# tum-vision/pnec

Hardware: AMD Instinct MI355X
Metric: PNEC pose solves/sec (512 corr, 10 GN iters) (higher is better)
Workload: dtype f64; 1 GPU; configs[1]: batch of 100k simulated frame pairs x 512 anisotropic-covariance correspondences per GPU; pairs_total=100000, launcher=single process, residual=PNEC target frame, setup_launches_before_warmup=15, pairs_per_gpu=100000, correspondences=512

## Files before the change

### pnec_amd/csrc/pnec_capi.hip

```cpp
#include <hip/hip_runtime.h>

#include <algorithm>
#include <cmath>
#include <cstdio>
#include <cstdlib>
#include <cstring>
#include <new>
#include <string>
#include <vector>

#include "pnec_batch_kernels.hpp"
#include "pnec_device.hpp"
#include "pnec_detect.hpp"
#include "pnec_front_shared.hpp"
#include "pnec_internal.hpp"
#include "pnec_keyframe.hpp"
#include "pnec_patch_cov.hpp"
#include "pnec_patch_store.hpp"
#include "pnec_patch_track.hpp"
#include "pnec_pose_cov.hpp"
#include "pnec_residuals.hpp"
#include "pnec_eight_point.hpp"
#include "pnec_undistort.hpp"
#include "pnec_trajectory.hpp"
// ... 526 lines not shown
    const std::string msg = g_last_error;
    pnec_hip_problem_destroy(p);
    g_last_error = msg;
    return rc;
  }
  *out = p;
  return 0;
}

int pnec_hip_problem_create(int device, int mode, int64_t n_pairs, const int64_t *offsets,
                            pnec_hip_problem **out) {
  return problem_create_impl(device, mode, 0, 0, n_pairs, offsets, out);
}

int pnec_hip_problem_create_capacity(int device, int mode, int64_t max_pairs, int64_t max_corr,
                                     pnec_hip_problem **out) {
  if (!out) return fail(PNEC_HIP_ERR_INVALID_ARGUMENT, "out is NULL");
  *out = nullptr;
  if (mode < PNEC_HIP_MODE_NEC || mode > PNEC_HIP_MODE_SYM) return fail(PNEC_HIP_ERR_INVALID_ARGUMENT, "unknown mode");
  if (max_pairs < 1 || max_corr < 0 || max_corr > (int64_t)1 << 40)
    return fail(PNEC_HIP_ERR_INVALID_ARGUMENT, "need max_pairs >= 1, max_corr >= 0");
  const int64_t cap_doubles = (int64_t)num_components(mode) * ((max_corr + 63 * max_pairs + kWave - 1) & ~(int64_t)(kWave - 1));
  const int64_t zero = 0;
  return problem_create_impl(device, mode, max_pairs, cap_doubles, 0, &zero, out);
}

int pnec_hip_problem_reshape(pnec_hip_problem *p, int64_t n_pairs, const int64_t *offsets, void *stream_) {
  return problem_reshape_impl(p, n_pairs, offsets, (hipStream_t)stream_, true);
}

int pnec_hip_problem_destroy(pnec_hip_problem *p) {
  if (!p) return 0;
  DeviceGuard guard(p->device);
  const bool drained = hipDeviceSynchronize() == hipSuccess;
  auto release = [&](void *ptr) { (void)(drained ? dev_free_drained(ptr) : dev_free(ptr)); };
  for (pnec_hip_problem *v : p->chunk_views) pnec_hip_problem_destroy(v);
  for (pnec_hip_problem *v : p->chunk_sel_views) pnec_hip_problem_destroy(v);
  if (p->sel_view) pnec_hip_problem_destroy(p->sel_view);
  if (p->nec_view) pnec_hip_problem_destroy(p->nec_view);
  release(p->d_mask);
  if (p->owns_data) {
    release(p->d_data);
    if (p->d_meta) {
      release(p->d_meta);
    } else {
      release(p->d_block_offset);
      release(p->d_offsets);
      release(p->d_count);
    }
  }
  release(p->d_stage);
  release(p->d_stage_i);
  release(p->d_ratio);
  release(p->d_front);
  release(p->d_front_i);
  release(p->d_hint_its);
  release(p->d_order);
  for (hipStream_t st : p->side_streams) {
    if (drained) pool_stream_put(st, p->device); else (void)hipStreamDestroy(st);
  }
  for (hipEvent_t ev : p->side_done) {
    if (drained) pool_event_put(ev, p->device); else (void)hipEventDestroy(ev);
  }
  for (hipStream_t st : p->chunk_streams) {
    if (drained) pool_stream_put(st, p->device); else (void)hipStreamDestroy(st);
  }
  for (hipEvent_t ev : p->chunk_done) {
    if (drained) pool_event_put(ev, p->device); else (void)hipEventDestroy(ev);
  }
  if (p->fork_event) {
    if (drained) pool_event_put(p->fork_event, p->device); else (void)hipEventDestroy(p->fork_event);
  }
  if (p->meta_uploaded) {
    if (drained) pool_event_put(p->meta_uploaded, p->device); else (void)hipEventDestroy(p->meta_uploaded);
  }
  if (p->bound_uploaded) {
    if (drained) pool_event_put(p->bound_uploaded, p->device); else (void)hipEventDestroy(p->bound_uploaded);
  }
  release(p->d_bound);
  release(p->d_bucket_pairs);
  release(p->d_fill);
  delete p;
  return 0;
}

int pnec_hip_problem_fill(pnec_hip_problem *p, int64_t first_pair, int64_t n_pairs,
                          const double *bvs1, const double *bvs2, const double *covs,
                          const double *covs_host, int space, void *stream_) {
  if (!p) return fail(PNEC_HIP_ERR_INVALID_ARGUMENT, "problem is NULL");
  if (first_pair < 0 || n_pairs < 0 || first_pair + n_pairs > p->n_pairs)
    return fail(PNEC_HIP_ERR_INVALID_ARGUMENT, "pair range out of bounds");
  if (n_pairs == 0) return 0;
  if (int rc = materialize(p)) return rc;
  const int64_t m = p->offsets[(size_t)(first_pair + n_pairs)] - p->offsets[(size_t)first_pair];
  if (m > 0 && (!bvs1 || !bvs2)) return fail(PNEC_HIP_ERR_INVALID_ARGUMENT, "bvs1/bvs2 is NULL");
  if (m > 0 && p->nc >= 12 && !covs)
    return fail(PNEC_HIP_ERR_INVALID_ARGUMENT, "covs is NULL for a PNEC-mode problem");
  if (m > 0 && p->nc >= 18 && !covs_host)
    return fail(PNEC_HIP_ERR_INVALID_ARGUMENT, "covs_host is NULL for a SYM-mode problem");
  DeviceGuard guard(p->device);
  hipStream_t stream = (hipStream_t)stream_;

  const double *d_b1 = bvs1, *d_b2 = bvs2, *d_c = covs, *d_ch = covs_host;
  double *tmp = nullptr;
  bool persistent_stage = false;
  if (space == PNEC_HIP_MEM_HOST && m > 0) {
// ... 297 lines not shown
  PNEC_HIP_TRY(launch_trajectory_metrics(a, stream));
  return io.finish();
}

int64_t pnec_hip_problem_payload_doubles(const pnec_hip_problem *p) { return p ? p->data_doubles : 0; }

int pnec_hip_problem_export_payload(const pnec_hip_problem *p, double *out, int space, void *stream_) {
  if (!p || !out) return fail(PNEC_HIP_ERR_INVALID_ARGUMENT, "NULL argument");
  if (space != PNEC_HIP_MEM_DEVICE && space != PNEC_HIP_MEM_HOST)
    return fail(PNEC_HIP_ERR_INVALID_ARGUMENT, "bad memory space");
  if (p->data_doubles == 0) return 0;
  DeviceGuard guard(p->device);
  hipStream_t stream = (hipStream_t)stream_;
  PNEC_HIP_TRY(hipMemcpyAsync(out, p->d_data, sizeof(double) * p->data_doubles,
                              space == PNEC_HIP_MEM_HOST ? hipMemcpyDeviceToHost : hipMemcpyDeviceToDevice, stream));
  if (space == PNEC_HIP_MEM_HOST) PNEC_HIP_TRY(hipStreamSynchronize(stream));
  return 0;
}

int64_t pnec_hip_problem_num_pairs(const pnec_hip_problem *p) { return p ? p->n_pairs : 0; }
int64_t pnec_hip_problem_num_correspondences(const pnec_hip_problem *p) {
  return p && materialize(p) == 0 ? p->n_corr : 0;
}
int64_t pnec_hip_problem_max_correspondences(const pnec_hip_problem *p) {
  return p && materialize(p) == 0 ? p->n_max : 0;
}
int64_t pnec_hip_problem_payload_bytes(const pnec_hip_problem *p) {
  return p && materialize(p) == 0 ? p->n_corr * p->nc * (int64_t)sizeof(double) : 0;
}
int pnec_hip_problem_offsets(const pnec_hip_problem *p, int64_t *out) {
  if (!p || !out) return fail(PNEC_HIP_ERR_INVALID_ARGUMENT, "NULL argument");
  if (int rc = materialize(p)) return rc;
  std::memcpy(out, p->offsets.data(), sizeof(int64_t) * p->offsets.size());
  return 0;
}
int pnec_hip_problem_mode(const pnec_hip_problem *p) { return p ? p->mode : -1; }
int pnec_hip_problem_device(const pnec_hip_problem *p) { return p ? p->device : -1; }

int pnec_hip_describe_launch(const pnec_hip_problem *p, const pnec_hip_options *opt,
                             int32_t *corr_per_lane, int32_t *waves_per_pair,
                             int32_t *lds_corr_per_lane, int32_t *threads_per_block,
                             int32_t *resident) {
  if (!p) return fail(PNEC_HIP_ERR_INVALID_ARGUMENT, "problem is NULL");
  Geometry g;
  if (int rc = choose_geometry(p, opt, &g)) return rc;
  if (corr_per_lane) *corr_per_lane = g.cpl;
  if (waves_per_pair) *waves_per_pair = g.wpp;
  if (lds_corr_per_lane) *lds_corr_per_lane = g.ldsk;
  if (threads_per_block) *threads_per_block = kWave * g.wpp;
  if (resident) *resident = g.resident ? 1 : 0;
  return 0;
}

int pnec_hip_solve(pnec_hip_problem *p, const double *init_q, const double *init_t, int32_t n_hyp,
                   const double *hyp_t, double reg, const pnec_hip_options *opt_in, double *out_q,
                   double *out_t, double *out_cost, int32_t *out_iterations, int32_t *out_status,
                   int space, void *stream_) {
  if (!p) return fail(PNEC_HIP_ERR_INVALID_ARGUMENT, "problem is NULL");
  if (!init_q) return fail(PNEC_HIP_ERR_INVALID_ARGUMENT, "init_q is NULL");
  if (!hyp_t) n_hyp = 1;
  if (n_hyp < 1) return fail(PNEC_HIP_ERR_INVALID_ARGUMENT, "n_hyp must be >= 1");
  if (!hyp_t && !init_t) return fail(PNEC_HIP_ERR_INVALID_ARGUMENT, "init_t and hyp_t are both NULL");
  if (int rc = check_space("", space)) return rc;
  pnec_hip_options opt;
  if (opt_in)
    opt = *opt_in;
  else
    pnec_hip_default_options(&opt);
  if (opt.max_num_iterations < 0) return fail(PNEC_HIP_ERR_INVALID_ARGUMENT, "max_num_iterations < 0");
  if (opt.flags & ~(PNEC_HIP_OPT_COUNT_PASSES | PNEC_HIP_OPT_JACOBIAN_NUMERIC_CENTRAL))
    return fail(PNEC_HIP_ERR_INVALID_ARGUMENT, "pnec_hip_options.flags: undefined bit set");
  const bool numeric = (opt.flags & PNEC_HIP_OPT_JACOBIAN_NUMERIC_CENTRAL) != 0;
  if (numeric) {
    opt.corr_per_lane = 0;
    opt.waves_per_pair = kStreamWaves;
    opt.lds_corr_per_lane = 0;
  }
  int64_t S;
  if (int rc = pose_slots(p, n_hyp, "solves", &S)) return rc;
  if (S == 0) return 0;
  Geometry g;
  if (int rc = choose_geometry(p, &opt, &g)) return rc;

  hipStream_t stream = (hipStream_t)stream_;
  CallArrays io(p, space, stream);
  SolveArgs a;
  std::memset(&a, 0, sizeof(a));
  a.data = p->d_data;
  a.block_offset = p->d_block_offset;
  a.count = p->d_count;
  a.n_solves = S;
  a.n_hyp = n_hyp;
  a.reg = reg;
  a.opt = opt;
  finish_args(a);
  a.numeric_jacobian = numeric ? 1 : 0;
  if (opt.flags & PNEC_HIP_OPT_COUNT_PASSES) {
    if (int rc = solve_work_buffer(p->device, &a.work)) return rc;
  }

  const int64_t P = p->n_pairs;
  io.in(a.init_q, init_q, 4 * P);
  io.in(a.init_t, init_t, 3 * P);
  io.in(a.hyp_t, hyp_t, 3 * S);
  io.out(a.out_q, out_q, 4 * S, kKeep);
  io.out(a.out_t, out_t, 3 * S, kKeep);
  io.out(a.out_cost, out_cost, S, kKeep);
  io.out(a.out_iterations, out_iterations, S, kKeep);
  io.out(a.out_status, out_status, S, kKeep);
  if (int rc = io.commit()) return rc;

  static const bool use_groups = [] {
    const char *ev = std::getenv("PNEC_SOLVE_GROUPS");
    return !(ev && *ev == '0');
  }();
  auto launch_on = [&](const Geometry &gg, const SolveArgs &aa, hipStream_t st) -> hipError_t {
    if (use_groups && aa.n_hyp > 1 && gg.resident && !aa.trace && !aa.numeric_jacobian &&
        (gg.wpp >= 2 ? group_geometry_ok(p->mode, gg.cpl, gg.wpp, gg.ldsk)
                     : pairhyp_geometry_ok(p->mode, gg.cpl, gg.wpp, gg.ldsk))) {
      switch (p->mode) {
        case PNEC_HIP_MODE_NEC: return launch_solve_group_mode_0(gg.cpl, gg.wpp, gg.ldsk, aa, st);
        case PNEC_HIP_MODE_TARGET: return launch_solve_group_mode_1(gg.cpl, gg.wpp, gg.ldsk, aa, st);
        case PNEC_HIP_MODE_HOST: return launch_solve_group_mode_2(gg.cpl, gg.wpp, gg.ldsk, aa, st);
        default: return launch_solve_group_mode_3(gg.cpl, gg.wpp, gg.ldsk, aa, st);
      }
    }
    switch (p->mode) {
      case PNEC_HIP_MODE_NEC: return launch_solve_mode_0(gg.cpl, gg.wpp, gg.ldsk, gg.resident, aa, st);
      case PNEC_HIP_MODE_TARGET: return launch_solve_mode_1(gg.cpl, gg.wpp, gg.ldsk, gg.resident, aa, st);
      case PNEC_HIP_MODE_HOST: return launch_solve_mode_2(gg.cpl, gg.wpp, gg.ldsk, gg.resident, aa, st);
      default: return launch_solve_mode_3(gg.cpl, gg.wpp, gg.ldsk, gg.resident, aa, st);
    }
  };
  auto launch = [&](const Geometry &gg, const SolveArgs &aa) -> hipError_t { return launch_on(gg, aa, stream); };
  const char *trace_path = std::getenv("PNEC_HIP_TRACE");
  unsigned long long *d_trace = nullptr;
  const bool forced = opt.corr_per_lane > 0 || opt.waves_per_pair > 0;
  if (!forced) {
    if (int rc = ensure_buckets(p)) return rc;
  }
  if (trace_path && *trace_path) {
    PNEC_HIP_TRY(dev_alloc(&d_trace, sizeof(unsigned long long) * 4 * S));
    const hipError_t te = hipMemsetAsync(d_trace, 0, sizeof(unsigned long long) * 4 * S, stream);
    if (te != hipSuccess) {
      (void)dev_free(d_trace);
      return fail_hip(te, "hipMemsetAsync(trace)");
    }
    a.trace = d_trace;
  }
  hipError_t e = hipSuccess;
  if (forced || p->buckets.size() <= 1) {
    e = launch(g, a);
  } else {
    const size_t n_side = p->buckets.size() - 1;
    if (int rc = ensure_side_streams(p, n_side)) {
      if (d_trace) (void)dev_free(d_trace);
      return rc;
    }
    e = hipEventRecord(p->fork_event, stream);
    for (size_t b = 0; b < p->buckets.size() && e == hipSuccess; ++b) {
      const auto &bk = p->buckets[b];
      SolveArgs ab = a;
      ab.pair_index = p->d_bucket_pairs + bk.first;
// ... 1307 lines not shown
```

### pnec_amd/csrc/pnec_internal.hpp

```cpp
#pragma once

#include <hip/hip_runtime.h>
#include <stdint.h>

#include <cstring>
#include <optional>
#include <string>
#include <type_traits>
#include <vector>

#include "pnec_call_plan.hpp"
#include "pnec_hip.h"

struct pnec_hip_problem {
  int device = 0;
  int mode = 0;
  int nc = 0;
  int64_t n_pairs = 0;
  int64_t n_corr = 0;
  int32_t n_max = 0;
  int64_t data_doubles = 0;
  int64_t cap_pairs = 0, cap_doubles = 0;
  uint64_t layout_gen = 0, view_src_gen = ~0ull;
  std::vector<int64_t> block_offset_host;
  std::vector<int64_t> meta_host;
  hipEvent_t meta_uploaded = nullptr;
  std::vector<int64_t> offsets;
  double *d_data = nullptr;
  int64_t *d_block_offset = nullptr;
  int64_t *d_offsets = nullptr;
  int32_t *d_count = nullptr;
  void *d_meta = nullptr;
  double *d_stage = nullptr;
  int64_t stage_doubles = 0;
  int32_t *d_stage_i = nullptr;
  int64_t stage_ints = 0;
  double *d_ratio = nullptr;
  int64_t ratio_doubles = 0;
  double *d_front = nullptr;
  int32_t *d_front_i = nullptr;
  int64_t front_pairs = 0;
  int es_scheme = 0;
  int ransac_flags = 0;
  double *d_fill = nullptr;
  int64_t fill_doubles = 0;
  bool order_hint = false;
  int32_t *d_hint_its = nullptr, *d_order = nullptr;
  int64_t hint_cap = 0, order_pairs = 0;
  struct Bucket {
    int cpl, wpp, ldsk;
    bool resident;
    int64_t count;
    int64_t first;
  };
  std::vector<Bucket> buckets;
  int32_t *d_bucket_pairs = nullptr;
  std::vector<hipStream_t> side_streams;
  std::vector<hipEvent_t> side_done;
  hipEvent_t fork_event = nullptr;
  std::vector<int32_t> host_counts;
  bool lazy = false;
  hipStream_t lazy_stream = nullptr;
  std::vector<int64_t> bound_offsets;
  std::vector<int32_t> bound_counts;
  int32_t *d_bound = nullptr;
  hipEvent_t bound_uploaded = nullptr;
  bool owns_data = true;
  pnec_hip_problem *sel_view = nullptr;
  pnec_hip_problem *nec_view = nullptr;
  std::vector<pnec_hip_problem *> chunk_views, chunk_sel_views;
  std::vector<hipStream_t> chunk_streams;
  std::vector<hipEvent_t> chunk_done;
  uint8_t *d_mask = nullptr;
  int64_t mask_bytes = 0;
};

namespace pnec_hip {

struct SolveArgs;

extern thread_local std::string g_last_error;
int fail(int code, const std::string &msg);
int fail_hip(hipError_t e, const char *what);
#define PNEC_HIP_TRY(expr)                                      \
  do {                                                          \
    hipError_t e_ = (expr);                                     \
    if (e_ != hipSuccess) return ::pnec_hip::fail_hip(e_, #expr); \
  } while (0)

hipError_t dev_alloc_bytes(void **out, size_t bytes);
template <typename T>
// ... 81 lines not shown
  int commit() {
    if (own_ && !guard_.ok) return fail(PNEC_HIP_ERR_HIP_RUNTIME, "hipSetDevice failed (no such device?)");
    if (slots_.empty()) return 0;
    if (int rc = ensure_stage(p_, plan_.doubles, plan_.ints)) return rc;
    for (size_t i = 0; i < slots_.size(); ++i) {
      const CallPlan::Entry &e = plan_.entries[i];
      Slot &s = slots_[i];
      if (e.room) s.dev = e.ints ? static_cast<void *>(p_->d_stage_i + e.offset) : static_cast<void *>(p_->d_stage + e.offset);
      std::memcpy(s.field, &s.dev, sizeof(void *));
      if (e.up && err_ == hipSuccess) err_ = hipMemcpyAsync(s.dev, s.caller, e.bytes, hipMemcpyHostToDevice, stream_);
    }
    return status();
  }
  int finish() {
    if (!host_) return 0;
    for (size_t i = 0; i < slots_.size(); ++i)
      if (plan_.entries[i].back && err_ == hipSuccess)
        err_ = hipMemcpyAsync(slots_[i].caller, slots_[i].dev, plan_.entries[i].bytes, hipMemcpyDeviceToHost, stream_);
    if (err_ == hipSuccess) err_ = hipStreamSynchronize(stream_);
    return status();
  }

 private:
  struct Slot {
    void *field;
    void *caller;
    void *dev;
  };
  template <typename F>
  void note(F &field, const void *caller, const CallPlan::Entry &) {
    static_assert(std::is_pointer<F>::value, "a field is a pointer");
    slots_.push_back({&field, const_cast<void *>(caller), nullptr});
  }
  int status() const { return err_ == hipSuccess ? 0 : fail_hip(err_, "host staging copy"); }
  DeviceGuard guard_;
  std::optional<pnec_hip_problem> own_;
  pnec_hip_problem *p_ = nullptr;
  bool host_;
  hipStream_t stream_;
  hipError_t err_ = hipSuccess;
  CallPlan plan_;
  std::vector<Slot> slots_;
};

hipError_t launch_solve_mode_0(int, int, int, bool, const SolveArgs &, hipStream_t);
hipError_t launch_solve_mode_1(int, int, int, bool, const SolveArgs &, hipStream_t);
hipError_t launch_solve_mode_2(int, int, int, bool, const SolveArgs &, hipStream_t);
hipError_t launch_solve_mode_3(int, int, int, bool, const SolveArgs &, hipStream_t);
hipError_t launch_solve_group_mode_0(int, int, int, const SolveArgs &, hipStream_t);
hipError_t launch_solve_group_mode_1(int, int, int, const SolveArgs &, hipStream_t);
hipError_t launch_solve_group_mode_2(int, int, int, const SolveArgs &, hipStream_t);
hipError_t launch_solve_group_mode_3(int, int, int, const SolveArgs &, hipStream_t);

hipError_t launch_solve_aos_mode_0(int, int, int, const SolveArgs &, hipStream_t);
hipError_t launch_solve_aos_mode_1(int, int, int, const SolveArgs &, hipStream_t);
hipError_t launch_solve_aos_mode_2(int, int, int, const SolveArgs &, hipStream_t);
hipError_t launch_solve_aos_mode_3(int, int, int, const SolveArgs &, hipStream_t);

hipError_t launch_ransac_eigensolver(const double *, const int64_t *, const int64_t *, const int32_t *, int64_t,
                                     const double *, unsigned long long, unsigned long long, int, int, double, double *, double *,
                                     uint8_t *, int32_t *, int32_t *, double *, int32_t *, hipStream_t, hipStream_t,
                                     hipEvent_t, hipEvent_t, int, double *, const int64_t *, int32_t *, int64_t *, const int32_t *, int, int);
hipError_t launch_ransac_order(const int32_t *, int64_t, int32_t *, hipStream_t);
hipError_t frontend_work_counters(int, unsigned long long *, int *);
hipError_t launch_select(int, const double *, const int64_t *, const int64_t *, const int32_t *, const uint8_t *,
                         double *, const int64_t *, const int32_t *, int32_t *, int64_t *, int64_t, hipStream_t);
hipError_t launch_nec_eigensolver(const double *, const int64_t *, const int32_t *, int64_t, const double *,
                                  double *, double *, int32_t *, double *, int32_t *, hipStream_t, int);
hipError_t launch_weighted_eigensolver(int, const double *, const int64_t *, const int32_t *, int64_t, int,
                                       const double *, const double *, double, int, double *, double *,
                                       int32_t *, double *, int32_t *, hipStream_t, int);
hipError_t launch_frontend_selftest(double *, hipStream_t);

}
```

### pnec_amd/csrc/pnec_solve_group_kernel.hpp

```cpp
#pragma once

#include "pnec_solve_kernel.hpp"

namespace pnec_hip {

constexpr int kGroupSub = 2;

#define PNEC_FOR_EACH_GROUP_GEOMETRY(X) X(4, 2, 0) X(4, 4, 0) X(4, 8, 0) X(8, 2, 3) X(8, 4, 3) X(8, 8, 3)
__host__ __device__ constexpr bool group_geometry_listed(int cpl, int wpp, int ldsk) {
#define PNEC_GROUP_MATCH(CPL, WPP, LDSK) if (cpl == CPL && wpp == WPP && ldsk == LDSK) return true;
  PNEC_FOR_EACH_GROUP_GEOMETRY(PNEC_GROUP_MATCH)
#undef PNEC_GROUP_MATCH
  return false;
}
__host__ __device__ constexpr bool group_geometry_ok(int mode, int cpl, int wpp, int ldsk) {
  if (!group_geometry_listed(cpl, wpp, ldsk) || !geometry_ok(mode, cpl, wpp, ldsk)) return false;
  const int nc = num_components(mode);
  const long lds = (long)wpp * (ldsk * nc * kWave * 8) + (long)wpp * ((kSlab + kUnif) * 8 + kINumI * 4) +
                   2L * kGroupSub * wpp * kSumSlots * 8;
  return lds <= 160 * 1024;
}

template <int G>
__device__ __forceinline__ constexpr int group_hyp_of_wave(int wave) { return 2 * (wave % (G / 2)) + wave / (G / 2); }

template <int MODE, int CPL, int WPP, int LDSK>
__global__ __launch_bounds__(kWave *WPP, (CPL == 8 && LDSK == 0) ? 1 : 2) void lm_solve_group_kernel(const SolveArgs a) {
  constexpr int G = WPP;
  constexpr int NC = num_components(MODE);
  constexpr int REGK = CPL - LDSK;
  constexpr int SB = kGroupSub;
  static_assert(G % SB == 0, "the pass phase exchanges sums every SB poses");
  const int lane = threadIdx.x & (kWave - 1);
  const int wave = threadIdx.x >> 6;
  const int groups_per_pair = (a.n_hyp + G - 1) / G;
  const int64_t n_pairs_here = a.n_solves / a.n_hyp;
  const int64_t logical = xcd_contiguous_index(blockIdx.x, n_pairs_here * groups_per_pair);
  const int64_t pslot = logical / groups_per_pair;
  const int h0 = (int)(logical % groups_per_pair) * G;
  const int nh = (a.n_hyp - h0) < G ? (a.n_hyp - h0) : G;
  const int64_t pair = a.pair_index ? (int64_t)a.pair_index[pslot] : pslot;
  const double *__restrict__ base = a.data + a.block_offset[pair];
  const int n = a.count[pair];
  const int stride = (n + kWave - 1) & ~(kWave - 1);
  const pnec_hip_options &o = a.opt;
  const double reg = a.reg;

  __shared__ double slab_all[G][kSlab];
  __shared__ double unif_all[G][kUnif];
  __shared__ int ist_all[G][kINumI];
  __shared__ double xw[2][SB][WPP][kSumSlots];
  [[maybe_unused]] __shared__ double ldata[LDSK > 0 ? WPP : 1][LDSK > 0 ? LDSK : 1][NC][LDSK > 0 ? kWave : 1];

  double d[REGK][NC];
  load_resident<NC, CPL, REGK>(base, n, stride, wave * CPL * kWave, lane, d, &ldata[LDSK > 0 ? wave : 0][0][0][0]);
  int nslots = 0;
#pragma unroll
  for (int k = 0; k < CPL; ++k) nslots += (n > wave * CPL * kWave + slot_corr<CPL, REGK>(k, 0)) ? 1 : 0;

  const int hw = group_hyp_of_wave<G>(wave);
  if (lane == 0) {
    const int h = hw;
    double *slab = slab_all[h];
    int *ist = ist_all[h];
    if (h < nh) {
      const int64_t s = pair * a.n_hyp + h0 + h;
      double th, ph;
      const double *t0 = a.hyp_t ? a.hyp_t + 3 * s : a.init_t + 3 * pair;
      start_angles(t0[0], t0[1], t0[2], th, ph);
      double q[4];
#pragma unroll
      for (int k = 0; k < 4; ++k) {
        q[k] = a.init_q[pair * 4 + k];
        slab[kQc + k] = q[k];
      }
      slab[kThetaC] = th;
      slab[kPhiC] = ph;
      pose_uniforms(th, ph, q, unif_all[h]);
    }
    ist[kIIter] = 0;
    ist[kIFirst] = 1;
    ist[kIReuseDiag] = 0;
    ist[kINumInvalid] = 0;
    ist[kIStepOk] = 1;
    ist[kILast] = o.max_num_iterations <= 0 ? 1 : 0;
    ist[kIPark] = 0;
    ist[kITerm] = h < nh ? -1 : PNEC_HIP_TERM_MAX_ITERATIONS;
  }
  const double inv_max_radius = a.inv_max_radius, inv_min_radius = a.inv_min_radius;
  if constexpr (LDSK > 0) __builtin_amdgcn_s_waitcnt(0x0F70);
  __builtin_amdgcn_fence(__ATOMIC_RELEASE, "wavefront");
  __syncthreads();

  int parity = 0;
  int n_full_passes = 0, n_cost_passes = 0;
  for (;;) {
#pragma unroll 1
    for (int sb = 0; sb < G / SB; ++sb) {
#pragma unroll 1
      for (int j = 0; j < SB; ++j) {
        const int h = sb * SB + j;
        if (to_sgpr(ist_all[h][kITerm]) >= 0) continue;
        const double *unif = unif_all[h];
        PassUniforms U;
#pragma unroll
        for (int i = 0; i < 9; ++i) U.R[i] = to_sgpr(unif[i]);
#pragma unroll
        for (int i = 0; i < 3; ++i) U.t[i] = to_sgpr(unif[9 + i]);
#pragma unroll
        for (int i = 0; i < 3; ++i) U.bth[i] = to_sgpr(unif[12 + i]);
        U.bph[0] = -U.t[1];
        U.bph[1] = U.t[0];
        U.bph[2] = 0.0;
        double c[6];
        const bool cost_only = to_sgpr(ist_all[h][kILast]) != 0;
        n_cost_passes += cost_only ? 1 : 0;
        n_full_passes += cost_only ? 0 : 1;
        if (cost_only) {
// ... 34 lines not shown
      const int t = lm_advance<true>(slab_all[hw], ist_all[hw], unif_all[hw], o, inv_max_radius, inv_min_radius);
      if (lane == 0) ist_all[hw][kITerm] = t;
    }
    __builtin_amdgcn_fence(__ATOMIC_RELEASE, "wavefront");
    __syncthreads();
    bool going = false;
#pragma unroll
    for (int h = 0; h < G; ++h) going = going || to_sgpr(ist_all[h][kITerm]) < 0;
    if (!going) break;
  }

  if (lane == 0 && hw < nh)
    write_result(a, pair * a.n_hyp + h0 + hw, slab_all[hw], ist_all[hw][kIIter], ist_all[hw][kITerm]);
  if (threadIdx.x == 0 && a.work) {
    atomicAdd(a.work + 0, (unsigned long long)n_full_passes * (unsigned long long)n);
    atomicAdd(a.work + 1, (unsigned long long)n_cost_passes * (unsigned long long)n);
  }
}

constexpr int kPairHyp = 2;
#define PNEC_FOR_EACH_PAIRHYP_GEOMETRY(X) X(1, 1, 0) X(2, 1, 0) X(4, 1, 0) X(8, 1, 3) X(8, 1, 0)
__host__ __device__ constexpr bool pairhyp_geometry_ok(int mode, int cpl, int wpp, int ldsk) {
  if (wpp != 1 || !geometry_ok(mode, cpl, wpp, ldsk)) return false;
#define PNEC_PH_MATCH(CPL, WPP, LDSK) if (cpl == CPL && ldsk == LDSK) return true;
  PNEC_FOR_EACH_PAIRHYP_GEOMETRY(PNEC_PH_MATCH)
#undef PNEC_PH_MATCH
  return false;
}

template <int MODE, int CPL, int LDSK>
__global__ __launch_bounds__(kWave, (CPL == 8 && LDSK == 0) ? 1 : 2) void lm_solve_pairhyp_kernel(const SolveArgs a) {
  constexpr int G = kPairHyp;
  constexpr int NC = num_components(MODE);
  constexpr int REGK = CPL - LDSK;
  const int lane = threadIdx.x;
  const int groups_per_pair = (a.n_hyp + G - 1) / G;
  const int64_t n_pairs_here = a.n_solves / a.n_hyp;
  const int64_t logical = xcd_contiguous_index(blockIdx.x, n_pairs_here * groups_per_pair);
  const int64_t pslot = logical / groups_per_pair;
  const int h0 = (int)(logical % groups_per_pair) * G;
  const int nh = (a.n_hyp - h0) < G ? (a.n_hyp - h0) : G;
  const int64_t pair = a.pair_index ? (int64_t)a.pair_index[pslot] : pslot;
  const double *__restrict__ base = a.data + a.block_offset[pair];
  const int n = a.count[pair];
  const int stride = (n + kWave - 1) & ~(kWave - 1);
  const pnec_hip_options &o = a.opt;
  const double reg = a.reg;

  __shared__ double slab_all[G][kSlab];
  __shared__ double unif_all[G][kUnif];
  __shared__ int ist_all[G][kINumI];
  [[maybe_unused]] __shared__ double ldata[LDSK > 0 ? LDSK : 1][NC][LDSK > 0 ? kWave : 1];

  double d[REGK][NC];
  load_resident<NC, CPL, REGK>(base, n, stride, 0, lane, d, &ldata[0][0][0]);
  int nslots = 0;
#pragma unroll
  for (int k = 0; k < CPL; ++k) nslots += (n > slot_corr<CPL, REGK>(k, 0)) ? 1 : 0;

  if ((lane & 3) == 0 && (lane >> 2) < G) {
    const int h = lane >> 2;
    double *slab = slab_all[h];
    int *ist = ist_all[h];
    if (h < nh) {
      const int64_t s = pair * a.n_hyp + h0 + h;
      double th, ph;
      const double *t0 = a.hyp_t ? a.hyp_t + 3 * s : a.init_t + 3 * pair;
      start_angles(t0[0], t0[1], t0[2], th, ph);
      double q[4];
#pragma unroll
      for (int k = 0; k < 4; ++k) {
        q[k] = a.init_q[pair * 4 + k];
        slab[kQc + k] = q[k];
      }
      slab[kThetaC] = th;
      slab[kPhiC] = ph;
      pose_uniforms(th, ph, q, unif_all[h]);
    }
    ist[kIIter] = 0;
    ist[kIFirst] = 1;
    ist[kIReuseDiag] = 0;
    ist[kINumInvalid] = 0;
    ist[kIStepOk] = 1;
    ist[kILast] = o.max_num_iterations <= 0 ? 1 : 0;
    ist[kIPark] = 0;
    ist[kITerm] = h < nh ? -1 : PNEC_HIP_TERM_MAX_ITERATIONS;
  }
  const double inv_max_radius = a.inv_max_radius, inv_min_radius = a.inv_min_radius;
  if constexpr (LDSK > 0) __builtin_amdgcn_s_waitcnt(0x0F70);
  auto wave_sync = [&]() {
    __builtin_amdgcn_fence(__ATOMIC_RELEASE, "wavefront");
    __builtin_amdgcn_wave_barrier();
    __builtin_amdgcn_fence(__ATOMIC_ACQUIRE, "wavefront");
  };
  wave_sync();

  int n_full_passes = 0, n_cost_passes = 0;
  for (;;) {
#pragma unroll 1
    for (int h = 0; h < G; ++h) {
      if (to_sgpr(ist_all[h][kITerm]) >= 0) continue;
      const double *unif = unif_all[h];
      PassUniforms U;
#pragma unroll
      for (int i = 0; i < 9; ++i) U.R[i] = to_sgpr(unif[i]);
#pragma unroll
      for (int i = 0; i < 3; ++i) U.t[i] = to_sgpr(unif[9 + i]);
#pragma unroll
      for (int i = 0; i < 3; ++i) U.bth[i] = to_sgpr(unif[12 + i]);
      U.bph[0] = -U.t[1];
      U.bph[1] = U.t[0];
      U.bph[2] = 0.0;
      double c[6];
      const bool cost_only = to_sgpr(ist_all[h][kILast]) != 0;
      n_cost_passes += cost_only ? 1 : 0;
      n_full_passes += cost_only ? 0 : 1;
      if (cost_only) {
// ... 48 lines not shown
```

### pnec_amd/csrc/pnec_solve_kernel.hpp

```cpp
#pragma once

#include <type_traits>

#include "pnec_device.hpp"


#define PNEC_FOR_EACH_GEOMETRY(X) \
  X(1, 1, 0) X(2, 1, 0) X(4, 1, 0) X(4, 2, 0) X(4, 4, 0) X(4, 8, 0) \
  X(8, 1, 3) X(12, 1, 3) X(8, 2, 3) X(8, 4, 3) X(8, 8, 3) X(8, 1, 0) X(1, 8, 0)
#define PNEC_FOR_EACH_AOS_GEOMETRY(X) \
  X(1, 1, 0) X(2, 1, 0) X(4, 1, 0) X(4, 4, 0) X(4, 8, 0) X(8, 1, 3) X(8, 2, 3) X(8, 4, 3) X(8, 8, 3) X(8, 1, 0)
constexpr int kStreamWaves = 8;

namespace pnec_hip {

struct SolveArgs {
  const double *data;
  const int64_t *block_offset;
  const int32_t *count;
  const int32_t *pair_index;
  const double *init_q;
  const double *init_t;
  const double *hyp_t;
  double *out_q;
  double *out_t;
  double *out_cost;
  int32_t *out_iterations;
  int32_t *out_status;
  unsigned long long *trace;
  unsigned long long *work;
  int64_t n_solves;
  int32_t n_hyp;
  int32_t numeric_jacobian;
  const double *aos_bvs1, *aos_bvs2, *aos_covs, *aos_covs_host;
  const int64_t *aos_offsets;
  unsigned long long *done_counter;
  unsigned long long *host_flag;
  unsigned long long flag_value, n_blocks_total;
  double reg;
  double inv_max_radius;
  double inv_min_radius;
  pnec_hip_options opt;
};
inline void finish_args(SolveArgs &a) {
  a.inv_max_radius = 1.0 / a.opt.max_trust_region_radius;
  a.inv_min_radius = 1.0 / a.opt.min_trust_region_radius;
}

__device__ __forceinline__ int64_t xcd_contiguous_index(int64_t b, int64_t n) {
  const int64_t xcd = b & 7, q = n >> 3, r = n & 7;
  const int64_t base = (xcd < r) ? xcd * (q + 1) : r * (q + 1) + (xcd - r) * q;
  return base + (b >> 3);
}

enum : int {
  kQ = 0,
  kTheta = 4,
  kPhi = 5,
  kCost = 6,
  kXNorm = 7,
  kInvRadius = 8,
  kDec = 9,
  kModel = 10,
  kQc = 11,
  kThetaC = 15,
  kPhiC = 16,
  kDiag = 17,
  kScaleSq = 22,
  kInvScaleSq = 27,
  kGmax = 32,
  kSumsFinite = 33,
  kSums = 36,
  kTcur = 84,
  kSlab = 88
};
constexpr int kUnif = 18;
enum : int { kIIter = 0, kIFirst, kIReuseDiag, kINumInvalid, kIStepOk,
              kILast,
              kIPark,
              kITerm,
              kISpec = kITerm,
              kINumI = 8 };
constexpr int kNumFallbacks = 3;
enum : int { kSpModel = 0, kSpQc = 1, kSpThetaC = 5, kSpPhiC = 6, kSpValid = 7, kSpUnif = 8 , kSpecSlot = 24 };
static_assert(kQc - kModel == kSpQc && kThetaC - kModel == kSpThetaC && kPhiC - kModel == kSpPhiC, "slot layout = slab layout");

__host__ __device__ constexpr bool geometry_ok(int mode, int cpl, int wpp, int ldsk) {
  const int nc = num_components(mode);
  if (cpl == 12) return wpp == 1 && ldsk == 3 && nc <= 12;
  const long lds = (long)wpp * (ldsk * nc * kWave * 8 + (kSlab + kUnif) * 8 + kINumI * 4) + (wpp > 1 ? 2L * wpp * kSumSlots * 8 : 0) +
                   (wpp == 1 ? kNumFallbacks * kSpecSlot * 8 : 0);
  if (lds > 160 * 1024) return false;
  if (cpl == 8 && ldsk == 0) return nc <= 18;
  return nc * (cpl - ldsk) <= 72;
}


__device__ __forceinline__ double atan2_c(double y, double x) {
  if (y == 0.0) return copysign(signbit(x) ? 3.14159265358979311600e+00 : 0.0, y);
  return atan2_lean(y, x);
}
__device__ __forceinline__ void start_angles(double x, double y, double z, double &theta, double &phi) {
  const double n = sqrt(x * x + y * y + z * z);
  if (n == 0.0) {
    theta = 0.0;
    phi = 0.0;
    return;
  }
  theta = acos_lean(z / n);
  phi = (fabs(theta) < 1e-10) ? 0.0 : atan2_c(y / n, x / n);
}

template <int CPL, int REGK>
__host__ __device__ constexpr int slot_corr(int k, int lane) {
  if (CPL == 1) return lane;
  if (k < (REGK & ~1)) return 2 * kWave * (k / 2) + 2 * lane + (k & 1);
  return kWave * k + lane;
}

template <int NC, int CPL, int REGK>
__device__ __forceinline__ void load_resident(const double *__restrict__ base, int n, int stride,
                                              int first_corr, int lane, double (&d)[REGK][NC],
                                              double *lds ) {
  (void)n;
  if constexpr (CPL == 1) {
    const int idx = first_corr + lane;
    const bool in = idx < stride;
#pragma unroll
    for (int c = 0; c < NC; ++c) d[0][c] = in ? base[(int64_t)c * stride + idx] : 0.0;
  } else {
    using pair_t = __attribute__((ext_vector_type(2))) double;
    auto load_pair = [&](auto jc) {
      constexpr int j = decltype(jc)::value;
      const int idx = first_corr + 2 * kWave * j + 2 * lane;
      const bool in = idx < stride;
#pragma unroll
      for (int c = 0; c < NC; ++c) {
        pair_t v = {0.0, 0.0};
        if (in) v = *reinterpret_cast<const pair_t *>(base + (int64_t)c * stride + idx);
        d[2 * j][c] = v.x;
        d[2 * j + 1][c] = v.y;
      }
    };
    if constexpr (REGK >= 2) load_pair(std::integral_constant<int, 0>{});
    if constexpr (REGK >= 4) load_pair(std::integral_constant<int, 1>{});
    if constexpr (REGK >= 6) load_pair(std::integral_constant<int, 2>{});
    if constexpr (REGK >= 8) load_pair(std::integral_constant<int, 3>{});
    if constexpr (REGK & 1) {
      const int idx = first_corr + kWave * (REGK - 1) + lane;
      const bool in = idx < stride;
#pragma unroll
      for (int c = 0; c < NC; ++c) d[REGK - 1][c] = in ? base[(int64_t)c * stride + idx] : 0.0;
    }
    typedef __attribute__((address_space(3))) void lds_void;
    typedef const __attribute__((address_space(1))) void global_void;
#pragma unroll
    for (int k = REGK; k < CPL; ++k) {
      const int chunk = first_corr + kWave * k;
      if (chunk < stride) {
        static_assert(NC % 2 == 0, "the LDS slots are loaded two planes at a time");
        const int plane_half = lane >> 5, in_plane = 2 * (lane & (kWave / 2 - 1));
#pragma unroll
        for (int c = 0; c < NC; c += 2)
          __builtin_amdgcn_global_load_lds((global_void *)(base + (int64_t)(c + plane_half) * stride + chunk + in_plane),
                                           (lds_void *)(uintptr_t)(uint32_t)(uintptr_t)(lds + ((k - REGK) * NC + c) * kWave),
// ... 549 lines not shown

#ifdef PNEC_ISA_MARKS
#define PNEC_MARK(name) asm volatile("; PNEC_MARK " name)
#else
#define PNEC_MARK(name)
#endif

constexpr int SRC_PLANES = 0;
constexpr int SRC_AOS = 1;
template <int MODE, int CPL, int WPP, int LDSK, bool RESIDENT, int SRC = SRC_PLANES>
__global__ __launch_bounds__(kWave *WPP, (CPL == 8 && LDSK == 0) ? 1 : 2) void lm_solve_kernel(const SolveArgs a) {
  static_assert(SRC != SRC_AOS || RESIDENT, "the AoS source is only built for the on-chip-resident geometries");
  constexpr int NC = num_components(MODE);
  constexpr int RCPL = CPL > 8 ? 8 : CPL;
  constexpr int TAILK = CPL - RCPL;
  static_assert(TAILK == 0 || (TAILK == 4 && WPP == 1 && RESIDENT && SRC != SRC_AOS), "the tail form is (12, 1, 3) on the batch's planes");
  constexpr int REGK = RESIDENT ? RCPL - LDSK : 1;
  const int lane = threadIdx.x & (kWave - 1);
  const int wave = threadIdx.x >> 6;
  const int64_t slot = xcd_contiguous_index(blockIdx.x, a.n_solves);
  const int64_t pair = a.pair_index ? (int64_t)a.pair_index[slot / a.n_hyp] : slot / a.n_hyp;
  const int64_t s = pair * a.n_hyp + slot % a.n_hyp;
  const double *__restrict__ base = nullptr;
  int n;
  int64_t aos0 = 0;
  if constexpr (SRC == SRC_AOS) {
    aos0 = a.aos_offsets[pair];
    n = (int)(a.aos_offsets[pair + 1] - aos0);
  } else {
    base = a.data + a.block_offset[pair];
    n = a.count[pair];
  }
  const int stride = (n + kWave - 1) & ~(kWave - 1);
  const pnec_hip_options &o = a.opt;
  const double reg = a.reg;

  unsigned long long t_begin = 0, t_loaded = 0;
  if (a.trace) t_begin = __builtin_amdgcn_s_memtime();

  __shared__ double slab_all[WPP][kSlab];
  __shared__ double unif_all[WPP][kUnif];
  __shared__ int ist_all[WPP][kINumI];
  constexpr int NFB = (WPP == 1 && RESIDENT && CPL == 8 && LDSK == 3) ? kNumFallbacks : 0;
  [[maybe_unused]] __shared__ double spec_all[NFB > 0 ? WPP : 1][NFB > 0 ? NFB * kSpecSlot : 1];
  [[maybe_unused]] __shared__ double xw[2][WPP > 1 ? WPP : 1][kSumSlots];
  [[maybe_unused]] __shared__ double nunif[RESIDENT ? 1 : kNumPoses][12];
  [[maybe_unused]] __shared__ double ninv2h[8];
  [[maybe_unused]] __shared__ double ldata[LDSK > 0 ? WPP : 1][LDSK > 0 ? LDSK : 1][NC][LDSK > 0 ? kWave : 1];
  double *slab = slab_all[WPP > 1 ? 0 : wave];
  double *unif = unif_all[WPP > 1 ? 0 : wave];
  int *ist = ist_all[WPP > 1 ? 0 : wave];
  [[maybe_unused]] int parity = 0;

  double d[REGK][NC];
  if constexpr (RESIDENT && SRC == SRC_AOS)
    load_resident_aos<NC, RCPL, REGK>(a.aos_bvs1 + 3 * aos0, a.aos_bvs2 + 3 * aos0, NC >= 12 ? a.aos_covs + 9 * aos0 : nullptr,
                                     NC >= 18 ? a.aos_covs_host + 9 * aos0 : nullptr, n, wave * RCPL * kWave, lane, d,
                                     &ldata[LDSK > 0 ? wave : 0][0][0][0]);
  else if constexpr (RESIDENT)
    load_resident<NC, RCPL, REGK>(base, n, stride, wave * RCPL * kWave, lane, d, &ldata[LDSK > 0 ? wave : 0][0][0][0]);
  [[maybe_unused]] int nslots = 0;
  if constexpr (RESIDENT) {
#pragma unroll
    for (int k = 0; k < RCPL; ++k) nslots += (n > wave * RCPL * kWave + slot_corr<RCPL, REGK>(k, 0)) ? 1 : 0;
  }
  [[maybe_unused]] int ntail = 0;
  [[maybe_unused]] const char *tail_base = nullptr;
  [[maybe_unused]] size_t tail_plane_bytes = 0;
  if constexpr (TAILK > 0) {
#pragma unroll
    for (int t = 0; t < TAILK; ++t) ntail += (n > RCPL * kWave + 2 * kWave * (t / 2) + (t & 1)) ? 1 : 0;
    const unsigned long long b64 = reinterpret_cast<unsigned long long>(base) + (unsigned long long)RCPL * kWave * sizeof(double);
    const unsigned blo = (unsigned)__builtin_amdgcn_readfirstlane((int)(unsigned)b64);
    const unsigned bhi = (unsigned)__builtin_amdgcn_readfirstlane((int)(unsigned)(b64 >> 32));
    tail_base = reinterpret_cast<const char *>(((unsigned long long)bhi << 32) | blo);
    tail_plane_bytes = (size_t)(unsigned)__builtin_amdgcn_readfirstlane(stride) * sizeof(double);
    ntail = __builtin_amdgcn_readfirstlane(ntail);
  }
  if (a.trace) {
    __builtin_amdgcn_s_waitcnt(0);
    t_loaded = __builtin_amdgcn_s_memtime();
  }

  if (lane == 0 && (WPP == 1 || wave == 0)) {
    double th, ph;
    const double *t0 = a.hyp_t ? a.hyp_t + 3 * s : a.init_t + 3 * pair;
    start_angles(t0[0], t0[1], t0[2], th, ph);
    double q[4];
#pragma unroll
    for (int k = 0; k < 4; ++k) {
      q[k] = a.init_q[pair * 4 + k];
      slab[kQc + k] = q[k];
    }
    slab[kThetaC] = th;
    slab[kPhiC] = ph;
    pose_uniforms(th, ph, q, unif);
    ist[kIIter] = 0;
    ist[kIFirst] = 1;
    ist[kIReuseDiag] = 0;
    ist[kINumInvalid] = 0;
    ist[kIStepOk] = 1;
    ist[kILast] = o.max_num_iterations <= 0 ? 1 : 0;
    ist[kIPark] = 0;
    if constexpr (WPP == 1) ist[kISpec] = kNumFallbacks;
  }
  const double inv_max_radius = a.inv_max_radius, inv_min_radius = a.inv_min_radius;
  if constexpr (RESIDENT && LDSK > 0 && SRC != SRC_AOS) __builtin_amdgcn_s_waitcnt(0x0F70);
  __builtin_amdgcn_fence(__ATOMIC_RELEASE, "wavefront");
  if constexpr (WPP > 1) __syncthreads();

  int term;
  int n_full_passes = 0, n_cost_passes = 0;
  for (;;) {
    PNEC_MARK("uniforms");
    {
      __builtin_amdgcn_fence(__ATOMIC_ACQUIRE, "wavefront");
      PassUniforms U;
#pragma unroll
      for (int i = 0; i < 9; ++i) U.R[i] = to_sgpr(unif[i]);
#pragma unroll
      for (int i = 0; i < 3; ++i) U.t[i] = to_sgpr(unif[9 + i]);
#pragma unroll
      for (int i = 0; i < 3; ++i) U.bth[i] = to_sgpr(unif[12 + i]);
      U.bph[0] = -U.t[1];
      U.bph[1] = U.t[0];
      U.bph[2] = 0.0;
      double c[6];
      bool cost_only = false;
      if constexpr (RESIDENT) cost_only = to_sgpr(ist[kILast]) != 0;
      n_cost_passes += cost_only ? 1 : 0;
      n_full_passes += cost_only ? 0 : 1;
      if (cost_only) {
        PNEC_MARK("pass_cost");
        if constexpr (RESIDENT) {
          double a0 = 0.0, z = 0.0;
          pass_cost_resident<MODE, REGK, LDSK>(d, &ldata[LDSK > 0 ? wave : 0][0][0][0], nslots, lane, U, reg,
                                               a0, z);
          c[0] = wave_reduce_acc0_row0(a0);
          c[1] = __builtin_amdgcn_ballot_w64(!(z == 0.0)) == 0ull ? 0.0 : __builtin_nan("");
          c[2] = c[3] = c[4] = c[5] = 0.0;
          if constexpr (TAILK > 0) {
            if (ntail > 0) {
              double a1 = 0.0, z1 = 0.0;
              const char *tb = tail_base;
              const size_t plane_bytes = tail_plane_bytes;
              const unsigned voff = 16u * (unsigned)lane;
              auto tail_cost = [&](auto tc) {
                constexpr int t = decltype(tc)::value;
                constexpr unsigned imm = 2u * kWave * 8u * (t / 2) + 8u * (t & 1);
// ... 171 lines not shown
```

Before: 37.95 million solves/s.

## Precompute per-solve start pose records in a separate kernel before the solve

Adds a lightweight pre-kernel that computes the starting angles, quaternion and pose uniforms for every solve and writes them to a padded 24-double record buffer. The solve kernels then load these records in parallel across lanes into LDS before the correspondence load, instead of having lane 0 serially run start_angles and pose_uniforms. The goal is to take the serial trig and uniform setup off the solve kernel's critical path. The cost is an extra launch and a global buffer round trip. It is on by default once there are at least 8192 solves.

```diff
diff --git a/pnec_amd/csrc/pnec_capi.hip b/pnec_amd/csrc/pnec_capi.hip
--- a/pnec_amd/csrc/pnec_capi.hip
+++ b/pnec_amd/csrc/pnec_capi.hip
@@ -602,6 +602,7 @@
   release(p->d_stage);
   release(p->d_stage_i);
   release(p->d_ratio);
+  release(p->d_start);
   release(p->d_front);
   release(p->d_front_i);
   release(p->d_hint_its);
@@ -1005,6 +1006,8 @@
   return 0;
 }
 
+constexpr int64_t kStartLaunchMinSolves = 8192;
+
 int pnec_hip_solve(pnec_hip_problem *p, const double *init_q, const double *init_t, int32_t n_hyp,
                    const double *hyp_t, double reg, const pnec_hip_options *opt_in, double *out_q,
                    double *out_t, double *out_cost, int32_t *out_iterations, int32_t *out_status,
@@ -1062,6 +1065,26 @@
   io.out(a.out_iterations, out_iterations, S, kKeep);
   io.out(a.out_status, out_status, S, kKeep);
   if (int rc = io.commit()) return rc;
+
+  static const int start_mode = [] {
+    const char *ev = std::getenv("PNEC_SOLVE_START");
+    if (ev && std::strcmp(ev, "kernel") == 0) return 1;
+    if (ev && std::strcmp(ev, "launch") == 0) return 2;
+    return 0;
+  }();
+  if (start_mode == 2 || (start_mode == 0 && S >= kStartLaunchMinSolves)) {
+    const int64_t need = S * (int64_t)kStartRecord;
+    if (need > p->start_doubles) {
+      if (p->d_start) (void)dev_free(p->d_start);
+      p->d_start = nullptr;
+      p->start_doubles = 0;
+      PNEC_HIP_TRY(dev_alloc(&p->d_start, sizeof(double) * (size_t)need));
+      p->start_doubles = need;
+    }
+    const hipError_t se = launch_solve_start(a.init_q, a.init_t, a.hyp_t, S, n_hyp, p->d_start, stream);
+    if (se != hipSuccess) return fail_hip(se, "solve_start_kernel launch");
+    a.start = p->d_start;
+  }
 
   static const bool use_groups = [] {
     const char *ev = std::getenv("PNEC_SOLVE_GROUPS");
diff --git a/pnec_amd/csrc/pnec_internal.hpp b/pnec_amd/csrc/pnec_internal.hpp
--- a/pnec_amd/csrc/pnec_internal.hpp
+++ b/pnec_amd/csrc/pnec_internal.hpp
@@ -37,6 +37,8 @@
   int64_t stage_ints = 0;
   double *d_ratio = nullptr;
   int64_t ratio_doubles = 0;
+  double *d_start = nullptr;
+  int64_t start_doubles = 0;
   double *d_front = nullptr;
   int32_t *d_front_i = nullptr;
   int64_t front_pairs = 0;
@@ -224,6 +226,9 @@
 hipError_t launch_solve_group_mode_2(int, int, int, const SolveArgs &, hipStream_t);
 hipError_t launch_solve_group_mode_3(int, int, int, const SolveArgs &, hipStream_t);
 
+hipError_t launch_solve_start(const double *init_q, const double *init_t, const double *hyp_t, int64_t n_solves,
+                              int32_t n_hyp, double *start, hipStream_t stream);
+
 hipError_t launch_solve_aos_mode_0(int, int, int, const SolveArgs &, hipStream_t);
 hipError_t launch_solve_aos_mode_1(int, int, int, const SolveArgs &, hipStream_t);
 hipError_t launch_solve_aos_mode_2(int, int, int, const SolveArgs &, hipStream_t);
diff --git a/pnec_amd/csrc/pnec_solve_group_kernel.hpp b/pnec_amd/csrc/pnec_solve_group_kernel.hpp
--- a/pnec_amd/csrc/pnec_solve_group_kernel.hpp
+++ b/pnec_amd/csrc/pnec_solve_group_kernel.hpp
@@ -52,18 +52,22 @@
   __shared__ double xw[2][SB][WPP][kSumSlots];
   [[maybe_unused]] __shared__ double ldata[LDSK > 0 ? WPP : 1][LDSK > 0 ? LDSK : 1][NC][LDSK > 0 ? kWave : 1];
 
+  const int hw = group_hyp_of_wave<G>(wave);
+  const bool pre = a.start != nullptr;
+  if (pre && hw < nh && lane < kStartDoubles)
+    start_put(lane, a.start[(pair * a.n_hyp + h0 + hw) * kStartRecord + lane], slab_all[hw], unif_all[hw]);
+
   double d[REGK][NC];
   load_resident<NC, CPL, REGK>(base, n, stride, wave * CPL * kWave, lane, d, &ldata[LDSK > 0 ? wave : 0][0][0][0]);
   int nslots = 0;
 #pragma unroll
   for (int k = 0; k < CPL; ++k) nslots += (n > wave * CPL * kWave + slot_corr<CPL, REGK>(k, 0)) ? 1 : 0;
 
-  const int hw = group_hyp_of_wave<G>(wave);
   if (lane == 0) {
     const int h = hw;
     double *slab = slab_all[h];
     int *ist = ist_all[h];
-    if (h < nh) {
+    if (h < nh && !pre) {
       const int64_t s = pair * a.n_hyp + h0 + h;
       double th, ph;
       const double *t0 = a.hyp_t ? a.hyp_t + 3 * s : a.init_t + 3 * pair;
@@ -204,6 +208,14 @@
   __shared__ int ist_all[G][kINumI];
   [[maybe_unused]] __shared__ double ldata[LDSK > 0 ? LDSK : 1][NC][LDSK > 0 ? kWave : 1];
 
+  static_assert(G * kStartRecord <= kWave, "one lane per double of the block's records");
+  const bool pre = a.start != nullptr;
+  {
+    const int start_h = lane / kStartRecord, start_i = lane % kStartRecord;
+    if (pre && start_h < nh && start_i < kStartDoubles)
+      start_put(start_i, a.start[(pair * a.n_hyp + h0) * kStartRecord + lane], slab_all[start_h], unif_all[start_h]);
+  }
+
   double d[REGK][NC];
   load_resident<NC, CPL, REGK>(base, n, stride, 0, lane, d, &ldata[0][0][0]);
   int nslots = 0;
@@ -214,7 +226,7 @@
     const int h = lane >> 2;
     double *slab = slab_all[h];
     int *ist = ist_all[h];
-    if (h < nh) {
+    if (h < nh && !pre) {
       const int64_t s = pair * a.n_hyp + h0 + h;
       double th, ph;
       const double *t0 = a.hyp_t ? a.hyp_t + 3 * s : a.init_t + 3 * pair;
diff --git a/pnec_amd/csrc/pnec_solve_kernel.hpp b/pnec_amd/csrc/pnec_solve_kernel.hpp
--- a/pnec_amd/csrc/pnec_solve_kernel.hpp
+++ b/pnec_amd/csrc/pnec_solve_kernel.hpp
@@ -22,6 +22,7 @@
   const double *init_q;
   const double *init_t;
   const double *hyp_t;
+  const double *start;
   double *out_q;
   double *out_t;
   double *out_cost;
@@ -111,6 +112,18 @@
   phi = (fabs(theta) < 1e-10) ? 0.0 : atan2_c(y / n, x / n);
 }
 
+constexpr int kStartRecord = 24;
+constexpr int kStartDoubles = 21;
+static_assert(kThetaC == kQc + 4 && kPhiC == kQc + 5 && kStartDoubles == 6 + 15, "record layout = slab[kQc ..] | unif[0 .. 14]");
+__device__ __forceinline__ void start_put(int i, double v, double *slab, double *unif) {
+  if (i < kStartDoubles) *(i < 6 ? slab + kQc + i : unif + (i - 6)) = v;
+}
+__host__ __device__ constexpr bool start_records_ok(int mode, int cpl, int wpp, int ldsk) {
+  if (mode == PNEC_HIP_MODE_HOST && cpl == 12) return false;
+  if (mode == PNEC_HIP_MODE_SYM && wpp == 1 && ldsk == 0 && cpl >= 4) return false;
+  return true;
+}
+
 template <int CPL, int REGK>
 __host__ __device__ constexpr int slot_corr(int k, int lane) {
   if (CPL == 1) return lane;
@@ -766,6 +779,12 @@
   int *ist = ist_all[WPP > 1 ? 0 : wave];
   [[maybe_unused]] int parity = 0;
 
+  constexpr bool kStartRecords = SRC != SRC_AOS && (!RESIDENT || start_records_ok(MODE, CPL, WPP, LDSK));
+  const bool pre = kStartRecords && a.start != nullptr;
+  if constexpr (kStartRecords) {
+    if (pre && (WPP == 1 || wave == 0) && lane < kStartDoubles) start_put(lane, a.start[s * kStartRecord + lane], slab, unif);
+  }
+
   double d[REGK][NC];
   if constexpr (RESIDENT && SRC == SRC_AOS)
     load_resident_aos<NC, RCPL, REGK>(a.aos_bvs1 + 3 * aos0, a.aos_bvs2 + 3 * aos0, NC >= 12 ? a.aos_covs + 9 * aos0 : nullptr,
@@ -797,18 +816,20 @@
   }
 
   if (lane == 0 && (WPP == 1 || wave == 0)) {
-    double th, ph;
-    const double *t0 = a.hyp_t ? a.hyp_t + 3 * s : a.init_t + 3 * pair;
-    start_angles(t0[0], t0[1], t0[2], th, ph);
-    double q[4];
-#pragma unroll
-    for (int k = 0; k < 4; ++k) {
-      q[k] = a.init_q[pair * 4 + k];
-      slab[kQc + k] = q[k];
-    }
-    slab[kThetaC] = th;
-    slab[kPhiC] = ph;
-    pose_uniforms(th, ph, q, unif);
+    if (!pre) {
+      double th, ph;
+      const double *t0 = a.hyp_t ? a.hyp_t + 3 * s : a.init_t + 3 * pair;
+      start_angles(t0[0], t0[1], t0[2], th, ph);
+      double q[4];
+#pragma unroll
+      for (int k = 0; k < 4; ++k) {
+        q[k] = a.init_q[pair * 4 + k];
+        slab[kQc + k] = q[k];
+      }
+      slab[kThetaC] = th;
+      slab[kPhiC] = ph;
+      pose_uniforms(th, ph, q, unif);
+    }
     ist[kIIter] = 0;
     ist[kIFirst] = 1;
     ist[kIReuseDiag] = 0;
diff --git a/pnec_amd/csrc/pnec_solve_start.hip b/pnec_amd/csrc/pnec_solve_start.hip
--- /dev/null
+++ b/pnec_amd/csrc/pnec_solve_start.hip
@@ -0,0 +1,43 @@
+#include "pnec_internal.hpp"
+#include "pnec_solve_kernel.hpp"
+
+namespace pnec_hip {
+
+constexpr int kStartBlock = 256;
+
+__global__ __launch_bounds__(kStartBlock) void solve_start_kernel(const double *__restrict__ init_q,
+                                                                   const double *__restrict__ init_t,
+                                                                   const double *__restrict__ hyp_t, int64_t n_solves,
+                                                                   int32_t n_hyp, double *__restrict__ start) {
+  const int64_t s = (int64_t)blockIdx.x * kStartBlock + threadIdx.x;
+  if (s >= n_solves) return;
+  const int64_t pair = s / n_hyp;
+  double th, ph;
+  const double *t0 = hyp_t ? hyp_t + 3 * s : init_t + 3 * pair;
+  start_angles(t0[0], t0[1], t0[2], th, ph);
+  double q[4];
+#pragma unroll
+  for (int k = 0; k < 4; ++k) q[k] = init_q[pair * 4 + k];
+  double u[kUnif];
+  pose_uniforms(th, ph, q, u);
+  double *rec = start + s * kStartRecord;
+#pragma unroll
+  for (int k = 0; k < 4; ++k) rec[k] = q[k];
+  rec[4] = th;
+  rec[5] = ph;
+#pragma unroll
+  for (int i = 0; i < kStartDoubles - 6; ++i) rec[6 + i] = u[i];
+#pragma unroll
+  for (int i = kStartDoubles; i < kStartRecord; ++i) rec[i] = 0.0;
+}
+
+hipError_t launch_solve_start(const double *init_q, const double *init_t, const double *hyp_t, int64_t n_solves,
+                              int32_t n_hyp, double *start, hipStream_t stream) {
+  const int64_t blocks = (n_solves + kStartBlock - 1) / kStartBlock;
+  if (blocks <= 0 || blocks > 0x7fffffffLL) return hipErrorInvalidConfiguration;
+  hipLaunchKernelGGL(solve_start_kernel, dim3((unsigned)blocks), dim3(kStartBlock), 0, stream, init_q, init_t, hyp_t,
+                     n_solves, n_hyp, start);
+  return hipGetLastError();
+}
+
+}
```

Result: no change. 38.14 million solves/s, median of 2 (+0.5%).
